# TuragaLab/flybody

Measured on AMD Instinct MI355X. Metric: env steps/sec (whole node), walk_imitation 4096-batch random-action rollout, higher is better.
Workload: dtype f64

## Files before the change

flybody_amd/csrc/fb_constraint.hpp:

```cpp
#pragma once
#include "fb_types.hpp"
#include "fb_math.hpp"
#include "fb_smooth.hpp"
#include "fb_newton.hpp"

#define JIDX(side, s, r) (((r)*2 + (side))*FB_MAXCH + (s))
#define MINIMP ((real)0.0001)
#define MAXIMP ((real)0.9999)

template <typename real>
FBD real get_impedance(const real* si, real pos, real margin) {
  real s0 = fmin(MAXIMP, fmax(MINIMP, si[0])), s1 = fmin(MAXIMP, fmax(MINIMP, si[1]));
  real s2 = fmax((real)0, si[2]), s3 = fmin(MAXIMP, fmax(MINIMP, si[3])), s4 = fmax((real)1, si[4]);
  if (s0 == s1 || s2 <= FB_MINV) return (real)0.5*(s0 + s1);
  real x = fabs((pos - margin)/s2);
  if (x >= 1) return s1;
  if (x <= 0) return s0;
  real y;
  if (s4 == 1) y = x;
  else if (s4 == 2) y = (x <= s3) ? x*x/s3 : 1 - (1 - x)*(1 - x)/(1 - s3);
  else if (x <= s3) y = pow(x, s4) / pow(s3, s4 - 1);
  else y = 1 - pow(1 - x, s4) / pow(1 - s3, s4 - 1);
  return s0 + y*(s1 - s0);
}
// ... 55 lines not shown
  real coff[3] = {0, 0, 0}, cfr[9] = {0, 0, 0, 0, 0, 0, 0, 0, 0};
  if (lane < ncon) {
    p = w.con_pair()[lane];
    dist = w.con_dist()[lane];
#pragma unroll
    for (int k = 0; k < 3; k++) coff[k] = w.con_pos()[3*lane + k] - w.com()[k];
#pragma unroll
    for (int k = 0; k < 9; k++) cfr[k] = w.con_frame()[9*lane + k];
    incl = M.pair_margin[p] - M.pair_gap[p];
    if (dist < incl) dim = (M.pair_condim[p] == 1) ? 1 : 3;
  }
  int adr = nlimit + wave_excl_scan(dim, lane);
  bool over = dim > 0 && adr + dim > FB_MAXEFC_;
  unsigned long long ob = __ballot(over);
  int nefc = nlimit + wave_sum_i(dim);
  if (ob) {
    int first = __ffsll((long long)ob) - 1;
    nefc = __shfl(adr, first, 64);
    if (lane >= first) dim = 0;
  }
  if (lane < ncon) { w.con_efc()[lane] = dim ? adr : -1; w.con_dim()[lane] = dim; }
  int b1 = 0, b2 = 0;
  if (dim) {
    { const int pb = M.pair_body[p]; b1 = pb & 0xffff; b2 = pb >> 16; }
    real K, B, imp;
    kbi(M, M.pair_solref + 2*p, M.pair_solimp + 5*p, dist, incl, false, K, B, imp);
    real tran = M.body_invweight0[2*b1] + M.body_invweight0[2*b2];
    real R0 = fmax(FB_MINV, (1 - imp)*tran/imp);
    const real* fr = M.pair_friction + 5*p;
    real R1 = R0 / fmax(FB_MINV, M.impratio);
    real mu = fr[0]*sqrt(R1/R0);
    real R2 = R1*fr[0]*fr[0]/(fr[1]*fr[1]);
    const int l1 = M.body_chlen[b1], l2 = M.body_chlen[b2];
    const int eA = l1 > 0 ? M.body_chain[b1*FB_MAXCH + l1 - 1] : -1, eB = l2 > 0 ? M.body_chain[b2*FB_MAXCH + l2 - 1] : -1;
    for (int k = 0; k < dim; k++) {
      int r = adr + k;
      w.efc_type()[r] = (dim == 1) ? CN_FRICTIONLESS : CN_ELLIPTIC; w.efc_id()[r] = lane;
      w.efc_bA()[r] = b1; w.efc_bB()[r] = b2;
      w.efc_lA()[r] = l1; w.efc_lB()[r] = l2;
      w.efc_pos()[r] = dist; w.efc_margin()[r] = incl;
      w.efc_K()[r] = (k == 0) ? K : (real)0; w.efc_B()[r] = B; w.efc_imp()[r] = imp;
      const real Rk = (k == 0) ? R0 : (k == 1 ? R1 : R2);
      w.efc_R()[r] = Rk; w.efc_D()[r] = (real)1 / Rk;
      w.efc_mu()[r] = mu;
      w.efc_k()[r] = k; w.efc_s1()[r] = (dim == 1) ? (real)1 : fr[0]; w.efc_s2()[r] = (dim == 1) ? (real)1 : fr[1];
      w.efc_eA()[r] = eA; w.efc_eB()[r] = eB;
    }
  }
  {
    const int cb1 = b1, cb2 = b2;
    const int nitem = ncon*(2*FB_MAXCH);
    for (int t0 = 0; t0 < nitem; t0 += FB_WAVE) {
      const int t = t0 + lane;
      const int c = min(t/(2*FB_MAXCH), FB_WAVE - 1), rem = t - c*(2*FB_MAXCH), side = rem >= FB_MAXCH ? 1 : 0, sl = rem - side*FB_MAXCH;
      const int cdim = __shfl(dim, c, 64), cadr = __shfl(adr, c, 64);
      const int sb1 = __shfl(cb1, c, 64), sb2 = __shfl(cb2, c, 64);
      const int body = side ? sb2 : sb1;
      real off[3], fr[9];
#pragma unroll
      for (int k = 0; k < 3; k++) off[k] = __shfl(coff[k], c, 64);
#pragma unroll
      for (int k = 0; k < 9; k++) fr[k] = __shfl(cfr[k], c, 64);
      if (t < nitem && cdim && sl < M.body_chlen[body]) {
        const int len = M.body_chlen[body];
        const int dof = M.body_chain[body*FB_MAXCH + sl];
        real jp[3] = {0, 0, 0};
        const FB_LDS real* cp = w.lLD + 6*((sl < len) ? dof : 0);
        real cd[6];
#pragma unroll
        for (int k = 0; k < 6; k++) cd[k] = cp[k];
        if (sl < len) {
          real tt[3]; cross3(tt, cd, off);
          jp[0] = cd[3] + tt[0]; jp[1] = cd[4] + tt[1]; jp[2] = cd[5] + tt[2];
        }
        const real sgn = side ? (real)1 : (real)-1;
        for (int k = 0; k < cdim; k++) w.efc_J()[JIDX(side, sl, cadr + k)] = sgn*dot3(fr + 3*k, jp);
      }
    }
  }
  if (lane == 0) {
    if (nefc > w.istate()[IS_MAX_NEFC]) w.istate()[IS_MAX_NEFC] = nefc;
    if (nefc > 32) w.istate()[IS_N_GT32]++;
    if (nefc > 64) w.istate()[IS_N_GT64]++;
    w.istate()[IS_NEFC] = nefc; w.istate()[IS_NLIMIT] = nlimit; if (ob || nlimit > FB_MAXEFC_) { atomicOr(w.istate() + IS_WARN, (int)WARN_EFC_CAP); atomicOr(w.istate() + IS_WARN_EVER, (int)WARN_EFC_CAP); } }
  SYNC();
}

#define ARIDX(r, c) ((r)*((r) + 1)/2 + (c))

template <typename real, typename ARP>
FB_STAGE_B void d_build_AR(const DevModel<real>& M, const WS<real>& w, ARP AR, int nefc, int lane);

template <typename real>
FBD void project_row(const DevModel<real>& M, const WS<real>& w, int side, int r, int body, int len, const FB_LDS real* sd, real* y) {
  int chain[FB_MAXCH], rowadr[FB_MAXCH];
  load_chain(M, body, chain);
#pragma unroll
  for (int s = 0; s < FB_MAXCH; s++) { y[s] = (s < len) ? w.efc_J()[JIDX(side, s, r)] : (real)0; rowadr[s] = (int)w.lmadr()[chain[s]] + s; }
  const int chmax = M.chmax;
#pragma unroll
  for (int s = FB_MAXCH - 1; s >= 1; s--) {
    if (s < chmax) {
      const FB_LDS real* row = w.lLD + rowadr[s];
#pragma unroll
      for (int t = 0; t < s; t++) y[t] -= row[-t] * y[s];
    }
  }
#pragma unroll
  for (int s = 0; s < FB_MAXCH; s++) y[s] = (s < len) ? y[s]*sd[chain[s]] : (real)0;
}

template <int TRUNK, typename real, typename ARP>
FBD void ar_from_registers_t(const DevModel<real>& M, const WS<real>& w, ARP AR, int nefc, int lane, const real* yA, const real* yB, int bA, int bB, int lA, int lB) {
  const bool valid = lane < nefc;
  const int c = lane;
  const int* common = M.body_common; const int nb = M.nbody;
  int rbA = rdlane(bA, 0), rbB = rdlane(bB, 0);
  int cAA = common[rbA*nb + bA], cAB = common[rbA*nb + bB], cBA = common[rbB*nb + bA], cBB = common[rbB*nb + bB];
  const real Rc = valid ? w.efc_R()[c] : (real)0;
  real tr[TRUNK > 0 ? TRUNK : 1];
#pragma unroll
  for (int s = 0; s < TRUNK; s++) tr[s] = yA[s] + yB[s];
  for (int r = 0; r < nefc; r++) {
    int rlA = rdlane(lA, r), rlB = rdlane(lB, r);
    int cmAA = min(min(cAA, lA), rlA), cmAB = min(min(cAB, lB), rlA), cmBA = min(min(cBA, lA), rlB), cmBB = min(min(cBB, lB), rlB);
    if (r + 1 < nefc) {
      rbA = rdlane(bA, r + 1); rbB = rdlane(bB, r + 1);
      cAA = common[rbA*nb + bA]; cAB = common[rbA*nb + bB]; cBA = common[rbB*nb + bA]; cBB = common[rbB*nb + bB];
    }
    real acc = 0;
#pragma unroll
    for (int s = 0; s < TRUNK; s++) acc += rdlane(tr[s], r)*tr[s];
#pragma unroll
    for (int s0 = 0; s0 < FB_MAXCH; s0 += 4) {
      if (s0 + 4 > TRUNK && s0 < rlA) {
#pragma unroll
        for (int s = s0; s < s0 + 4; s++) if (s >= TRUNK) { real yr = rdlane(yA[s], r); if (s < cmAA) acc += yr*yA[s]; if (s < cmAB) acc += yr*yB[s]; }
      }
    }
#pragma unroll
    for (int s0 = 0; s0 < FB_MAXCH; s0 += 4) {
      if (s0 + 4 > TRUNK && s0 < rlB) {
#pragma unroll
        for (int s = s0; s < s0 + 4; s++) if (s >= TRUNK) { real yr = rdlane(yB[s], r); if (s < cmBA) acc += yr*yA[s]; if (s < cmBB) acc += yr*yB[s]; }
      }
    }
    if (valid && c <= r) {
      if (c == r) acc += Rc;
      AR[ARIDX(r, c)] = acc;
    }
  }
  SYNC();
}
template <typename real, typename ARP>
FBD void ar_from_registers(const DevModel<real>& M, const WS<real>& w, ARP AR, int nefc, int lane, const real* yA, const real* yB, int bA, int bB, int lA, int lB) {
  if (uniform_int(M.ntrunk) == FB_MAXTRUNK) ar_from_registers_t<FB_MAXTRUNK>(M, w, AR, nefc, lane, yA, yB, bA, bB, lA, lB);
  else
  ar_from_registers_t<0>(M, w, AR, nefc, lane, yA, yB, bA, bB, lA, lB);
}

template <typename real>
__device__ __forceinline__ void d_project_constraint(const DevModel<real>& M, const WS<real>& w, int lane) {
  int nefc = w.istate()[IS_NEFC];
  if (nefc == 0) return;
  FB_LDS real* sd = w.lx();
  for (int i = lane; i < M.nv; i += FB_WAVE) sd[i] = sqrt(w.lLD[w.lmadr()[i]]);
  SYNC();
  if (nefc <= FB_WAVE) {
    real yA[FB_MAXCH], yB[FB_MAXCH];
    int bA = 0, bB = 0, lA = 0, lB = 0;
    if (lane < nefc) { bA = w.efc_bA()[lane]; bB = w.efc_bB()[lane]; lA = w.efc_lA()[lane]; lB = w.efc_lB()[lane]; }
    project_row(M, w, 0, lane < nefc ? lane : 0, bA, lA, sd, yA);
    project_row(M, w, 1, lane < nefc ? lane : 0, bB, lB, sd, yB);
    if (nefc <= LdsCfg<real>::AR_ROWS) ar_from_registers(M, w, w.lAR(), nefc, lane, yA, yB, bA, bB, lA, lB);
    else ar_from_registers(M, w, w.AR(), nefc, lane, yA, yB, bA, bB, lA, lB);
    return;
  }
  for (int base = 0; base < nefc; base += FB_WAVE) {
    int r = base + lane;
    if (r < nefc) {
      for (int side = 0; side < 2; side++) {
        int body = side ? w.efc_bB()[r] : w.efc_bA()[r];
        int len = side ? w.efc_lB()[r] : w.efc_lA()[r];
        real y[FB_MAXCH];
        project_row(M, w, side, r, body, len, sd, y);
#pragma unroll
        for (int s = 0; s < FB_MAXCH; s++) w.efc_Y()[JIDX(side, s, r)] = y[s];
      }
    }
  }
  SYNC();
  const WS<real> wc = w;
  d_build_AR(M, wc, w.AR(), nefc, lane);
}

template <typename real, typename ARP>
FB_STAGE_B void d_build_AR(const DevModel<real>& M_, const WS<real>& w_, ARP AR, int nefc, int lane) {
  const DevModel<real>& M = as_constant(M_); const WS<real> w = ws_uniform(w_, M);
  for (int cbase = 0; cbase < nefc; cbase += FB_WAVE) {
    int c = cbase + lane;
    bool valid = c < nefc;
    real yA[FB_MAXCH], yB[FB_MAXCH];
    int bA = 0, bB = 0, lA = 0, lB = 0;
    if (valid) { bA = w.efc_bA()[c]; bB = w.efc_bB()[c]; lA = w.efc_lA()[c]; lB = w.efc_lB()[c]; }
#pragma unroll
    for (int s = 0; s < FB_MAXCH; s++) {
      yA[s] = valid ? w.efc_Y()[JIDX(0, s, c)] : (real)0;
      yB[s] = valid ? w.efc_Y()[JIDX(1, s, c)] : (real)0;
    }
    if (nefc <= FB_WAVE) {
      const int* common = M.body_common; const int nb = M.nbody;
      int rbA = rdlane(bA, 0), rbB = rdlane(bB, 0);
      int cAA = common[rbA*nb + bA], cAB = common[rbA*nb + bB], cBA = common[rbB*nb + bA], cBB = common[rbB*nb + bB];
      for (int r = 0; r < nefc; r++) {
        int rlA = rdlane(lA, r), rlB = rdlane(lB, r);
        int cmAA = min(min(cAA, lA), rlA), cmAB = min(min(cAB, lB), rlA), cmBA = min(min(cBA, lA), rlB), cmBB = min(min(cBB, lB), rlB);
        if (r + 1 < nefc) {
          rbA = rdlane(bA, r + 1); rbB = rdlane(bB, r + 1);
          cAA = common[rbA*nb + bA]; cAB = common[rbA*nb + bB]; cBA = common[rbB*nb + bA]; cBB = common[rbB*nb + bB];
        }
        real acc = 0;
#pragma unroll
        for (int s = 0; s < FB_MAXCH; s++) {
          if (s < rlA) { real yr = rdlane(yA[s], r); if (s < cmAA) acc += yr*yA[s]; if (s < cmAB) acc += yr*yB[s]; }
        }
#pragma unroll
        for (int s = 0; s < FB_MAXCH; s++) {
          if (s < rlB) { real yr = rdlane(yB[s], r); if (s < cmBA) acc += yr*yA[s]; if (s < cmBB) acc += yr*yB[s]; }
        }
        if (valid && c <= r) {
          if (c == r) acc += w.efc_R()[r];
          AR[ARIDX(r, c)] = acc;
        }
      }
    } else
    for (int r = 0; r < nefc; r++) {
      real acc = 0;
      for (int side = 0; side < 2; side++) {
        int rb = side ? w.efc_bB()[r] : w.efc_bA()[r];
        int rl = side ? w.efc_lB()[r] : w.efc_lA()[r];
        if (rl == 0) continue;
        int cmA = min(min(M.body_common[rb*M.nbody + bA], lA), rl);
        int cmB = min(min(M.body_common[rb*M.nbody + bB], lB), rl);
#pragma unroll
        for (int s = 0; s < FB_MAXCH; s++) {
          if (s < rl) {
            real yr = w.efc_Y()[JIDX(side, s, r)];
            if (s < cmA) acc += yr*yA[s];
            if (s < cmB) acc += yr*yB[s];
          }
        }
      }
      if (valid && c <= r) {
        if (c == r) acc += w.efc_R()[r];
        AR[ARIDX(r, c)] = acc;
      }
    }
  }
  SYNC();
}

template <typename real>
__device__ __forceinline__ void d_actuation(const DevModel<real>& M, const WS<real>& w, int lane) {
  FB_LDS real* qf = w.lx();
  FB_LDS real* Lc = w.lLD;
  for (int i = lane; i < M.nv; i += FB_WAVE) qf[i] = 0;
  SYNC_LDS();
  const int ncon_l = w.istate()[IS_NCON];
  int cb1 = 0, cb2 = 0, cp = 0;
  real coff[3] = {0, 0, 0}, cnrm[3] = {0, 0, 0};
  constexpr int NCD = (6*FB_MAXNV + FB_WAVE - 1)/FB_WAVE;
  real cdr[NCD];
  if (M.nadh > 0) {
    cp = w.con_pair()[lane];
#pragma unroll
    for (int k = 0; k < 3; k++) { coff[k] = w.con_pos()[3*lane + k]; cnrm[k] = w.con_frame()[9*lane + k]; }
#pragma unroll
    for (int j = 0; j < NCD; j++) { const int i = lane + FB_WAVE*j; cdr[j] = i < 6*M.nv ? w.cdof()[i] : (real)0; }
  }
  for (int i = lane; i < M.nu; i += FB_WAVE) {
    const int limited = M.act_ctrllimited[i], aa = M.act_actadr[i], tt = M.act_trntype[i], wn = M.act_wn[i], la = M.act_lenadr[i];
    const int biastype = M.act_biastype[i], flimited = M.act_forcelimited[i];
    const real c_lo = M.act_ctrlrange[2*i], c_hi = M.act_ctrlrange[2*i+1], dyn = M.act_dynprm[i], gain = M.act_gainprm[3*i];
    const real b0 = M.act_biasprm[3*i], b1 = M.act_biasprm[3*i+1], b2 = M.act_biasprm[3*i+2], f_lo = M.act_forcerange[2*i], f_hi = M.act_forcerange[2*i+1];
    int wd[FB_MAXWRAP]; real wc[FB_MAXWRAP], qv[FB_MAXWRAP];
#pragma unroll
    for (int k = 0; k < FB_MAXWRAP; k++) { wd[k] = M.act_wdof[FB_MAXWRAP*i + k]; wc[k] = M.act_wcoef[FB_MAXWRAP*i + k]; }
    real ctrl = w.ctrl()[i];
    const real actv = w.act()[aa >= 0 ? aa : 0];
#pragma unroll
    for (int k = 0; k < FB_MAXWRAP; k++) qv[k] = w.qvel()[wd[k]];
    const real lq = w.qpos()[tt == TRN_JOINT ? la : 0];
    const real lt = w.ten_length()[tt == TRN_TENDON ? la : 0];
    if (limited) ctrl = clampr(ctrl, c_lo, c_hi);
    real input = ctrl;
    if (aa >= 0) {
      w.act_dot()[aa] = (ctrl - actv) / fmax(FB_MINV, dyn);
      input = actv;
    }
    real length = 0, vel = 0;
    if (tt == TRN_JOINT) length = lq;
    else if (tt == TRN_TENDON) length = lt;
#pragma unroll
    for (int k = 0; k < FB_MAXWRAP; k++) if (k < wn) vel += wc[k]*qv[k];
    real force = gain*input;
    if (biastype == 1) force += b0 + b1*length + b2*vel;
    if (flimited) force = clampr(force, f_lo, f_hi);
    w.act_force()[i] = force;
#pragma unroll
    for (int k = 0; k < FB_MAXWRAP; k++) if (k < wn) qf[wd[k]] = wc[k]*force;
  }
// ... 637 lines not shown
```

flybody_amd/csrc/fb_engine.hip:

```cpp
#ifdef FB_EMULATE
#include "emu/hip_emu.hpp"
#else
#include <hip/hip_runtime.h>
#endif
#include <algorithm>
#include <cmath>
#include <cstdio>
#include <cstdlib>
#include <cstring>
#include <map>
#include <stdexcept>
#include <string>
#include <vector>
#if defined(FB_EMULATE) && defined(FB_STATS)
extern "C" { long long fb_stats[64]; }
#endif

#include "../../include/flybody_engine.h"
#include "fb_step.hpp"
#include "fb_ik.hpp"
#include "fb_inverse.hpp"

static thread_local std::string g_err;
static int fail(const std::string& s) { g_err = s; return -1; }
// ... 660 lines not shown
    int key = iarena[(size_t)(j*nq + xcc)*nint + off_nefc]; key = key < 0 ? 0 : (key > 255 ? 255 : key);
    atomicAdd(&s_hist[255 - key], 1);
  }
  __syncthreads();
  if (tid == 0) { int acc = 0; for (int k = 0; k < 256; k++) { int h = s_hist[k]; s_hist[k] = acc; acc += h; } }
  __syncthreads();
  for (int j = tid; j < cnt; j += FB_ORDER_THREADS) {
    const int e = j*nq + xcc;
    int key = iarena[(size_t)e*nint + off_nefc]; key = key < 0 ? 0 : (key > 255 ? 255 : key);
    order[xcc*stride + atomicAdd(&s_hist[255 - key], 1)] = e;
  }
}

FB_HD __forceinline__ void fb_philox4x32_10(uint32_t c0, uint32_t c1, uint32_t c2, uint32_t c3, uint32_t k0, uint32_t k1, uint32_t* out) {
  for (int r = 0; r < 10; r++) {
    const uint64_t p0 = (uint64_t)0xD2511F53u*c0, p1 = (uint64_t)0xCD9E8D57u*c2;
    const uint32_t n0 = (uint32_t)(p1 >> 32) ^ c1 ^ k0, n1 = (uint32_t)p1, n2 = (uint32_t)(p0 >> 32) ^ c3 ^ k1, n3 = (uint32_t)p0;
    c0 = n0; c1 = n1; c2 = n2; c3 = n3;
    k0 += 0x9E3779B9u; k1 += 0xBB67AE85u;
  }
  out[0] = c0; out[1] = c1; out[2] = c2; out[3] = c3;
}
__global__ void __launch_bounds__(FB_WAVE) k_actions(float* out, const int* env_ids, int n_env, int nact, uint32_t seed_lo, uint32_t seed_hi, int step, int env_id_base, int dist) {
  const int ngrp = (nact + 3)/4;
  const int t = blockIdx.x*FB_WAVE + threadIdx.x;
  if (t >= n_env*ngrp) return;
  const int e = t / ngrp, g = t - e*ngrp;
  const int gid = env_ids ? env_ids[e] : env_id_base + e;
  uint32_t r[4];
  fb_philox4x32_10((uint32_t)step, (uint32_t)gid, (uint32_t)g, (uint32_t)dist, seed_lo, seed_hi, r);
  float v[4];
  if (dist == 1) {
    for (int k = 0; k < 4; k++) v[k] = ((float)(r[k] >> 8) + 0.5f)*(2.0f/16777216.0f) - 1.0f;
  } else {
    for (int k = 0; k < 4; k += 2) {
      const float u1 = ((float)(r[k] >> 8) + 0.5f)*(1.0f/16777216.0f), u2 = ((float)(r[k + 1] >> 8) + 0.5f)*(1.0f/16777216.0f);
      const float rad = sqrtf(-2.0f*logf(u1)), ang = 6.28318530717958647692f*u2;
      v[k] = rad*cosf(ang); v[k + 1] = rad*sinf(ang);
    }
    for (int k = 0; k < 4; k++) v[k] = fminf(1.0f, fmaxf(-1.0f, v[k]));
  }
  for (int k = 0; k < 4; k++) if (4*g + k < nact) out[(size_t)e*nact + 4*g + k] = v[k];
}

extern "C" int fb_random_actions(float* action, const int32_t* env_ids, int n_env, int nact, uint64_t seed, int step, int env_id_base, int dist, void* stream) {
  if (!action || n_env <= 0 || nact <= 0 || (dist != 0 && dist != 1)) return fail("fb_random_actions: bad arguments");
  const int total = n_env*((nact + 3)/4);
  hipLaunchKernelGGL(k_actions, dim3((total + FB_WAVE - 1)/FB_WAVE), dim3(FB_WAVE), 0, (hipStream_t)stream, action, (const int*)env_ids, n_env, nact,
                     (uint32_t)(seed & 0xffffffffu), (uint32_t)(seed >> 32), step, env_id_base, dist);
  HIPCHK(hipGetLastError());
  return 0;
}

struct fb_batch {
  const fb_model* m;
  int n_env, device, precision, nobs;
  WSOff off;
  void* rarena = nullptr; int* iarena = nullptr;
  float *obs = nullptr, *reward = nullptr, *discount = nullptr; int* step_type = nullptr;
  int* d_ids = nullptr;
  int* sched = nullptr;
  int *cost = nullptr, *order = nullptr; bool order_valid = false, reorder = true, use_prio = true, ticket_order = true;
  int *tick = nullptr, *done = nullptr, *sched_err = nullptr, *torder = nullptr; int nq = 0, slots = 0; bool tickets = false;
  unsigned xcc_mask = 0; std::vector<void*> probed_streams; unsigned* probe_word = nullptr;
  void* park = nullptr;
  std::vector<void*> allocs;
  DevModel<double> M64; DevModel<float> M32;
  void* dM = nullptr;
  std::vector<char> dM_copy;
  void *ref_qpos = nullptr, *ref_qvel = nullptr;
  bool have_ref = false, have_wbpg = false;
  hipEvent_t ev0 = nullptr, ev1 = nullptr; int timed_launches = 0; bool timing = false;
  std::vector<hipEvent_t> lev;
  double* ik_err = nullptr; int* ik_steps = nullptr;
  void* ik_buf = nullptr; size_t ik_buf_bytes = 0;
  double* inv_qfrc = nullptr; double* inv_cforce = nullptr;
  void *qfrc_applied = nullptr, *xfrc_applied = nullptr;
};

template <typename real, typename T, typename P>
static int upload(fb_batch* b, const T* src, size_t n, P* dst) {
  std::vector<real> tmp(n ? n : 1);
  for (size_t k = 0; k < n; k++) tmp[k] = (real)src[k];
  void* p;
  HIPCHK(hipMalloc(&p, tmp.size()*sizeof(real)));
  HIPCHK(hipMemcpy(p, tmp.data(), tmp.size()*sizeof(real), hipMemcpyHostToDevice));
  b->allocs.push_back(p);
  *dst = (const real*)p;
  return 0;
}
template <typename P>
static int upload_i(fb_batch* b, const int* src, size_t n, P* dst) {
  void* p;
  HIPCHK(hipMalloc(&p, (n ? n : 1)*sizeof(int)));
  if (n) HIPCHK(hipMemcpy(p, src, n*sizeof(int), hipMemcpyHostToDevice));
  else HIPCHK(hipMemset(p, 0, sizeof(int)));
  b->allocs.push_back(p);
  *dst = (const int*)p;
  return 0;
}

template <typename F>
static auto with_model(fb_batch* b, F&& f) { return b->precision == 64 ? f(b->M64) : f(b->M32); }
static size_t real_size(fb_batch* b) { return with_model(b, [](auto& M) { return sizeof(M.timestep); }); }

static int sync_model(fb_batch* b) {
  return with_model(b, [&](auto& M) {
    if (!b->dM) HIPCHK(hipMalloc(&b->dM, sizeof(M)));
    const char* h = (const char*)&M;
    if (b->dM_copy.empty() || memcmp(h, b->dM_copy.data(), sizeof(M)) != 0) {
      HIPCHK(hipDeviceSynchronize());
      HIPCHK(hipMemcpy(b->dM, h, sizeof(M), hipMemcpyHostToDevice));
      b->dM_copy.assign(h, h + sizeof(M));
    }
    return 0;
  });
}

template <typename T>
static int alloc_zeroed_once(T** p, size_t bytes) {
  if (!*p) { HIPCHK(hipMalloc((void**)p, bytes)); HIPCHK(hipMemset(*p, 0, bytes)); }
  return 0;
}

static int alloc_obs(fb_batch* b, int nobs) {
  (void)hipFree(b->obs); b->obs = nullptr;
  HIPCHK(hipMalloc((void**)&b->obs, (size_t)b->n_env*nobs*sizeof(float)));
  HIPCHK(hipMemset(b->obs, 0, (size_t)b->n_env*nobs*sizeof(float)));
  b->nobs = nobs;
  return 0;
}

template <typename real>
static int build_devmodel(fb_batch* b, DevModel<real>& M) {
  const fb_model* m = b->m;
  memset(&M, 0, sizeof(M));
  M.nq = m->nq; M.nv = m->nv; M.nbody = m->nbody; M.njnt = m->njnt; M.ngeom = m->ngeom; M.nsite = m->nsite;
  M.nu = m->nu; M.na = m->na; M.ntendon = m->ntendon; M.npair = m->npair; M.nM = m->nM; M.nsubstep = m->nsubstep;
  M.nobsjnt = m->nobsjnt; M.napp = m->napp; M.nforce = m->nforce; M.ntouch = m->ntouch;
  M.site_thorax = m->i("sensor_site_thorax")[0]; M.nadh = (int)m->adh_act.size();
  M.iterations = m->i("opt_iterations")[0]; M.noslip_iterations = m->i("opt_noslip_iterations")[0];
  M.solver = (m->has("opt_solver", 1) && m->i("opt_solver")[0] == FB_SOLVER_PGS) ? FB_SOLVER_PGS : FB_SOLVER_NEWTON;
  M.timestep = (real)m->d("opt_timestep")[0]; M.control_timestep = (real)m->d("opt_control_timestep")[0];
  for (int k = 0; k < 3; k++) M.grav[k] = (real)m->d("opt_gravity")[k];
  M.density = (real)m->d("opt_density")[0]; M.viscosity = (real)m->d("opt_viscosity")[0];
  M.impratio = (real)m->d("opt_impratio")[0]; M.tolerance = (real)m->d("opt_tolerance")[0];
  {
    std::vector<double> rb; const double* r_ = m->d("geom_rbound");
    for (int g = 0; g < m->ngeom; g++) if (r_[g] > 0) rb.push_back(r_[g]);
    std::sort(rb.begin(), rb.end());
    M.vl_delta = (rb.empty() || m->npair <= 4*FB_WAVE) ? (real)0 : (real)(FB_VL_SCALE*rb[rb.size()/2]);
    { const char* e_ = getenv("FB_NO_NEIGHBOUR_LIST"); if (e_ && e_[0] == '1') M.vl_delta = 0; }
  }
  M.noslip_tolerance = (real)m->d("opt_noslip_tolerance")[0]; M.meaninertia = (real)m->d("stat_meaninertia")[0];
  M.totalmass = (real)m->totalmass;
  size_t c;
#define UI(field, name) { const int* s_ = m->i(name, &c); if (upload_i(b, s_, c, &M.field)) return -1; }
#define UV(field, vec) { if (upload_i(b, m->vec.data(), m->vec.size(), &M.field)) return -1; }
#define UD(field, name) { const double* s_ = m->d(name, &c); if (upload<real>(b, s_, c, &M.field)) return -1; }
  UI(body_parent, "body_parent") UI(body_dofadr, "body_dofadr")
  UV(body_nsub, body_nsub) UV(body_depth, body_depth) UV(body_chlen, body_chlen) UV(body_chain, body_chain) UV(body_common, body_common)
  UI(jnt_type, "jnt_type") UI(jnt_qposadr, "jnt_qposadr") UI(jnt_dofadr, "jnt_dofadr") UI(jnt_bodyid, "jnt_bodyid") UI(jnt_limited, "jnt_limited")
  UI(dof_bodyid, "dof_bodyid") UI(dof_jntid, "dof_jntid") UI(dof_Madr, "dof_Madr") UV(dof_depth, dof_depth)
  UV(dof_ndesc, dof_ndesc) UV(body_fluid_geom, body_fluid_geom) UV(sens_body, sens_body) M.nsensbody = (int)m->sens_body.size();
  UV(dof_jump, dof_jump) UV(dof_vbef, dof_vbef) UV(body_veldof, body_veldof)
  UV(dof_cl, dof_cl) UV(dof_gen, dof_gen) UV(gen_k, gen_k) UV(gen_m, gen_m) UV(fwd_tab, fwd_tab) UV(fwd_pack, fwd_pack) UV(fac_w, fac_w) UV(fac_band, fac_band) UV(fac_dof, fac_dof) M.ntrunk = m->ntrunk; M.prefix_split = m->prefix_split;
  { int dmax = 0, d2 = 1 << 20; for (int bq = 1; bq < m->nbody; bq++) { dmax = std::max(dmax, m->body_depth[bq]); if (bq >= FB_WAVE) d2 = std::min(d2, m->body_depth[bq]); } M.fk_dmax = dmax; M.fk2_dlo = d2; }
  { int cm = 0; for (int bq = 0; bq < m->nbody; bq++) cm = std::max(cm, m->body_chlen[bq]); M.chmax = cm; }
  {
    std::vector<int> second(FB_WAVE, -1);
    bool ok = m->nbody > FB_WAVE && m->nbody <= 2*FB_WAVE && getenv("FB_NO_FK_MERGE") == nullptr;
    for (int bq = FB_WAVE; ok && bq < m->nbody; bq++) {
      int pick = -1;
      for (int l = 0; l < FB_WAVE && pick < 0; l++) if (second[l] < 0 && (l == 0 || m->body_depth[l] < m->body_depth[bq])) pick = l;
      if (pick < 0) ok = false; else second[pick] = bq;
    }
    M.fk_second = nullptr;
    if (ok && upload_i(b, second.data(), second.size(), &M.fk_second)) return -1;
  }
  UI(wing_act_idx, "wing_action_idx")
  if (m->has("leg_joints", 1)) { UI(leg_jnt, "leg_joints") M.nlegjnt = (int)c; for (size_t k = 0; k < c; k++) if (m->i("leg_joints")[k] < 0 || m->i("leg_joints")[k] >= m->njnt) return fail("fb_batch_create: leg_joints out of range"); }
  else { UV(leg_jnt, adh_act) M.nlegjnt = 0; }
  M.task = m->task_id; M.user_idx = m->i("user_action_idx")[0]; M.nact = m->nu + (M.user_idx >= 0 ? 1 : 0);
  for (int k = 0; k < 3; k++) M.com_offset[k] = (real)m->d("com_offset")[k];
  M.nlevel = m->nlevel;
  UI(geom_type, "geom_type") UI(geom_bodyid, "geom_bodyid") UI(site_bodyid, "site_bodyid") UI(site_type, "site_type")
  UI(tendon_adr, "tendon_adr") UI(tendon_num, "tendon_num")
  UI(act_trntype, "actuator_trntype") UI(act_trnid, "actuator_trnid") UI(act_dyntype, "actuator_dyntype") UI(act_biastype, "actuator_biastype")
  UI(act_ctrllimited, "actuator_ctrllimited") UI(act_forcelimited, "actuator_forcelimited") UI(act_actadr, "actuator_actadr")
  UV(adh_act, adh_act) UI(action_to_ctrl, "action_to_ctrl")
  UV(wrap_qadr, wrap_qadr) UV(act_wn, act_wn) UV(act_wdof, act_wdof) UV(act_lenadr, act_lenadr)
  if (upload<real>(b, m->act_wcoef.data(), m->act_wcoef.size(), &M.act_wcoef)) return -1;
  UI(pair_geom1, "pair_geom1") UI(pair_geom2, "pair_geom2") UI(pair_condim, "pair_condim")
  UV(pair_word, pair_word) UV(pair_body, pair_body) UV(plane_geoms, plane_geoms)
  { const int* gt_ = m->i("geom_type"); int np_ = 0; for (int g = 0; g < m->ngeom; g++) np_ += gt_[g] == GEOM_PLANE; M.nplane = np_; }
  UI(obs_jnt, "observable_joints") UI(app_sites, "appendage_sites") UI(force_sites, "sensor_force_sites") UI(touch_sites, "sensor_touch_sites") UI(wing_jnt, "wing_jnt")
  UD(body_mass, "body_mass")
  UD(body_inertia, "body_inertia") UD(body_invweight0, "body_invweight0")
  if (upload<real>(b, m->body_box.data(), m->body_box.size(), &M.body_box)) return -1;
  if (upload<real>(b, m->geom_box.data(), m->geom_box.size(), &M.geom_box)) return -1;
  if (upload<real>(b, m->body_rec.data(), m->body_rec.size(), &M.body_rec)) return -1;
  UD(jnt_axis, "jnt_axis") UD(jnt_stiffness, "jnt_stiffness") UD(jnt_range, "jnt_range") UD(jnt_solref, "jnt_solref")
  UD(jnt_solimp, "jnt_solimp") UD(jnt_margin, "jnt_margin") UD(qpos0, "qpos0") UD(qpos_spring, "qpos_spring")
  UD(dof_armature, "dof_armature") UD(dof_damping, "dof_damping") UD(dof_invweight0, "dof_invweight0")
  UD(geom_pos, "geom_pos") UD(geom_quat, "geom_quat") UD(geom_size, "geom_size") UD(geom_rbound, "geom_rbound") UD(geom_fluid, "geom_fluid")
  UD(site_pos, "site_pos") UD(site_quat, "site_quat") UD(site_size, "site_size") UD(wrap_coef, "wrap_coef")
  UD(act_dynprm, "actuator_dynprm") UD(act_gainprm, "actuator_gainprm") UD(act_biasprm, "actuator_biasprm") UD(act_ctrlrange, "actuator_ctrlrange") UD(act_forcerange, "actuator_forcerange")
  UD(pair_friction, "pair_friction") UD(pair_solref, "pair_solref") UD(pair_solimp, "pair_solimp") UD(pair_margin, "pair_margin") UD(pair_gap, "pair_gap")
#undef UI
#undef UV
#undef UD
  return 0;
}

template <typename real>
static void compute_offsets(const DevModel<real>& M, WSOff& o) {
  uint32_t r = 0, i = 0;
  auto al = [](uint32_t v) { return (v + 15u) & ~15u; };
#define X(name, n) o.name = r; r = al(r + (uint32_t)(n));
  FB_WS_REAL(X)
#undef X
#define X(name, n) o.name = i; i = al(i + (uint32_t)(n));
  FB_WS_INT(X)
#undef X
  o.nreal = (r + 15u) & ~15u; o.nint = (i + 15u) & ~15u;
}

static int batch_create_impl(fb_batch* b);

extern "C" int fb_batch_create(const fb_model* m, int n_env, int device, int precision, fb_batch** out) {
  if (!out) return fail("fb_batch_create: null output pointer");
  *out = nullptr;
  if (!m || n_env <= 0) return fail("fb_batch_create: bad arguments");
  if (precision != 32 && precision != 64) return fail("fb_batch_create: precision must be 32 or 64");
  int ndev = 0;
  if (hipGetDeviceCount(&ndev) != hipSuccess || ndev <= 0) return fail("fb_batch_create: no HIP device available (the engine has no CPU fallback)");
  if (device < 0 || device >= ndev) return fail("fb_batch_create: bad device index");
  HIPCHK(hipSetDevice(device));
  fb_batch* b = new fb_batch();
  b->m = m; b->n_env = n_env; b->device = device; b->precision = precision;
  int rc;
  try { rc = batch_create_impl(b); } catch (const std::exception& e_) { rc = fail(std::string("fb_batch_create: ") + e_.what()); }
  if (rc != 0) { std::string keep = g_err; fb_batch_destroy(b); g_err = keep; return rc; }
  *out = b;
  return 0;
}

static int batch_create_impl(fb_batch* b) {
  const fb_model* m = b->m; const int n_env = b->n_env;
  if (with_model(b, [&](auto& M) { if (build_devmodel(b, M)) return -1; compute_offsets(M, b->off); M.off = b->off; return 0; })) return -1;
  const size_t rs = real_size(b);
  HIPCHK(hipMalloc(&b->rarena, (size_t)n_env*b->off.nreal*rs));
  HIPCHK(hipMemset(b->rarena, 0, (size_t)n_env*b->off.nreal*rs));
  HIPCHK(hipMalloc((void**)&b->iarena, (size_t)n_env*b->off.nint*sizeof(int)));
  HIPCHK(hipMemset(b->iarena, 0, (size_t)n_env*b->off.nint*sizeof(int)));
  HIPCHK(hipMalloc((void**)&b->reward, n_env*sizeof(float)));
  HIPCHK(hipMalloc((void**)&b->discount, n_env*sizeof(float)));
  HIPCHK(hipMalloc((void**)&b->step_type, n_env*sizeof(int)));
  HIPCHK(hipMalloc((void**)&b->d_ids, n_env*sizeof(int)));
  HIPCHK(hipMalloc((void**)&b->sched, FB_NSCHED*sizeof(int)));
  HIPCHK(hipMalloc((void**)&b->cost, n_env*sizeof(int)));
  HIPCHK(hipMemset(b->cost, 0, n_env*sizeof(int)));
  HIPCHK(hipMalloc((void**)&b->order, n_env*sizeof(int)));
  { const char* e_ = getenv("FB_NO_REORDER"); b->reorder = !(e_ && e_[0] == '1'); b->ticket_order = b->reorder; }
  {
#ifdef FB_EMULATE
    b->nq = 1; b->slots = 2;
#else
    hipDeviceProp_t prop; HIPCHK(hipGetDeviceProperties(&prop, b->device));
    if (with_model(b, [&](auto& M) {
          using real = decltype(M.timestep);
          int nb = 0;
          HIPCHK(hipOccupancyMaxActiveBlocksPerMultiprocessor(&nb, k_fly<real>, FB_WAVE*LdsCfg<real>::EPB, 0));
          int nbf = 0;
          HIPCHK(hipOccupancyMaxActiveBlocksPerMultiprocessor(&nbf, k_step_forces<real>, FB_WAVE*LdsCfg<real>::EPB, 0));
          b->slots = std::min(nb, nbf)*prop.multiProcessorCount*LdsCfg<real>::EPB;
          return 0; })) return -1;
    unsigned* dmask; unsigned hmask = 0;
    HIPCHK(hipMalloc((void**)&dmask, sizeof(unsigned))); HIPCHK(hipMemset(dmask, 0, sizeof(unsigned)));
    hipLaunchKernelGGL(k_probe_xcc, dim3(4096), dim3(FB_WAVE), 0, 0, dmask);
    HIPCHK(hipMemcpy(&hmask, dmask, sizeof(unsigned), hipMemcpyDeviceToHost)); HIPCHK(hipFree(dmask));
    int nqq = __builtin_popcount(hmask);
    b->nq = (nqq > 0 && hmask == (1u << nqq) - 1u) ? nqq : 0;
    b->xcc_mask = hmask;
    if (strncmp(prop.gcnArchName, "gfx942", 6) != 0 && strncmp(prop.gcnArchName, "gfx950", 6) != 0) b->nq = 0;
    if (const char* e_ = getenv("FB_TICKET_SLOTS")) b->slots = atoi(e_);
#endif
    HIPCHK(hipMalloc((void**)&b->tick, 16*16*sizeof(int)));
    HIPCHK(hipMalloc((void**)&b->done, n_env*sizeof(int)));
    HIPCHK(hipMalloc((void**)&b->torder, (size_t)(n_env + 16)*sizeof(int)));
    HIPCHK(hipMalloc((void**)&b->sched_err, sizeof(int)));
    HIPCHK(hipMemset(b->sched_err, 0, sizeof(int)));
    HIPCHK(hipMalloc((void**)&b->probe_word, sizeof(unsigned)));
    b->tickets = b->nq > 0 && b->slots > 0 && n_env > b->slots && getenv("FB_NO_TICKETS") == nullptr;
  }
  b->use_prio = getenv("FB_NO_PRIO") == nullptr;
  HIPCHK(hipMemset(b->reward, 0, n_env*sizeof(float)));
  HIPCHK(hipMemset(b->discount, 0, n_env*sizeof(float)));
  HIPCHK(hipMemset(b->step_type, 0, n_env*sizeof(int)));
  if (with_model(b, [&](auto& M) {
        std::vector<decltype(M.timestep)> rows((size_t)n_env*m->nq);
        const double* q0 = m->d("qpos0");
        for (int e = 0; e < n_env; e++) std::copy_n(q0, m->nq, rows.data() + (size_t)e*m->nq);
        HIPCHK(hipMemcpy2D((char*)b->rarena + (size_t)b->off.qpos*rs, (size_t)b->off.nreal*rs, rows.data(), (size_t)m->nq*rs, (size_t)m->nq*rs, n_env, hipMemcpyHostToDevice));
        return 0; })) return -1;
  b->nobs = 0;
// ... 601 lines not shown
```

flybody_amd/csrc/fb_types.hpp:

```cpp
#pragma once
#ifdef FB_EMULATE
#include "emu/hip_emu.hpp"
#else
#include <hip/hip_runtime.h>
#endif
#include <stdint.h>

#if defined(FB_EMULATE) && defined(FB_STATS)
extern "C" { extern long long fb_stats[64]; }
#define FB_STAT(k) (fb_stats[k]++)
#else
#define FB_STAT(k) do {} while (0)
#endif

#define FB_WAVE 64
#define FB_EPB 4
#define FB_MAXCH 20
#define FB_MAXGEN 16
#define FB_LDS_SCRATCH 1216
#define FB_LGEN 6
#define FB_BODYREC 40
#define FB_MAXTRUNK 6
#define FB_FSLOT 18
#define FB_FGEN 2
#define FB_MAXDEPTH 10
#define FB_MAXCON_ 64
#define FB_MAXEFC_ 192
#define FB_NSENS 33
#define FB_NWS_VECS 18
#define FB_NPROF 56
#define FB_NSCHED 64
#define FB_MAXWRAP 8
#define FB_MAXNM 1280
#define FB_MAXNV 112
#define FB_NJUMP 5

enum { JNT_FREE = 0, JNT_BALL = 1, JNT_HINGE = 3 };
enum { GEOM_PLANE = 0, GEOM_SPHERE = 2, GEOM_CAPSULE = 3, GEOM_ELLIPSOID = 4, GEOM_CYLINDER = 5 };
enum { TRN_JOINT = 0, TRN_TENDON = 3, TRN_BODY = 5 };
enum { DYN_NONE = 0, DYN_FILTER = 2, DYN_FILTEREXACT = 3 };
enum { CN_LIMIT = 0, CN_FRICTIONLESS = 1, CN_ELLIPTIC = 2 };
enum { IS_STEP = 0, IS_RESET_NEXT = 1, IS_STEP_TYPE = 2, IS_NCON = 3, IS_NEFC = 4, IS_NITER = 5, IS_NLIMIT = 6, IS_NCAND = 7,
       IS_WB_STEP = 8, IS_WB_FREQ = 9, IS_EPISODE = 10, IS_DS_OFF = 11, IS_DS_LEN = 12, IS_EPSTEPS = 13, IS_PRIO = 14, IS_WARN = 15, IS_WARN_EVER = 16,
       IS_MAX_NCON = 17, IS_MAX_NEFC = 18, IS_N_GT32 = 19, IS_N_GT64 = 20,
       IS_VL_OK = 21, IS_VL_N = 22, IS_VL_SKIP = 23,
       IS_N = 24 };
#define FB_VL_SCALE 0.5
#define FB_VLMAX 448
enum { WARN_CONTACT_CAP = 1, WARN_EFC_CAP = 2, WARN_SOLVER_MAXITER = 4, WARN_CCD_MAXITER = 8, WARN_SCHED_WAIT = 16, WARN_SOLVER_FALLBACK = 32 };


#if defined(__HIP_DEVICE_COMPILE__) && !defined(FB_EMULATE)
#define FB_GLOBAL __attribute__((address_space(1)))
#define FB_CONST __attribute__((address_space(4)))
#else
#define FB_GLOBAL
#define FB_CONST
#endif
#ifdef FB_EMULATE
#define FB_HD
#else
#define FB_HD __host__ __device__
#endif
template <typename T> struct GP {
  FB_GLOBAL T* p;
  FB_HD __forceinline__ operator T*() const { return (T*)p; }
  FB_HD __forceinline__ GP& operator=(T* q) { p = (FB_GLOBAL T*)q; return *this; }
};

#define FB_WS_REAL(X) \
  X(qpos, M.nq) X(qvel, M.nv) X(act, M.na + 1) X(ctrl, M.nu) X(qacc, M.nv) X(qacc_ws, M.nv) X(act_dot, M.na + 1) \
  X(sens, FB_NSENS) X(sens_acc, FB_NSENS) X(simtime, 1) X(wbfreq, 1) X(dsshift, 2) X(rfac, 6) \
  X(xpos, 3*M.nbody) X(xquat, 4*M.nbody)  \
  X(xaxis, 3*M.njnt)  X(gxpos, 3*M.ngeom) X(gxmat, 9*M.ngeom) X(sxpos, 3*M.nsite) X(sxmat, 9*M.nsite) X(com, 4) \
  X(cinert, 10*M.nbody) X(cdof, 6*M.nv) X(cvel, 6*M.nbody) \
  X(qM, M.nM) X(qLD, M.nM) \
  X(qfrc_bias, M.nv) X(qfrc_passive, M.nv) X(qfrc_actuator, M.nv) X(qfrc_smooth, M.nv) X(qacc_smooth, M.nv) \
  X(qfrc_constraint, M.nv) X(ten_length, M.ntendon + 1) X(act_force, M.nu) \
  X(con_dist, FB_MAXCON_) X(con_pos, 3*FB_MAXCON_) X(con_frame, 9*FB_MAXCON_) \
  X(efc_J, 2*FB_MAXCH*FB_MAXEFC_) \
  X(efc_pos, FB_MAXEFC_) X(efc_margin, FB_MAXEFC_) X(efc_R, FB_MAXEFC_) X(efc_D, FB_MAXEFC_) X(efc_K, FB_MAXEFC_) \
  X(efc_B, FB_MAXEFC_) X(efc_imp, FB_MAXEFC_) X(efc_aref, FB_MAXEFC_) X(efc_b, FB_MAXEFC_) X(efc_force, FB_MAXEFC_) \
  X(efc_vel, FB_MAXEFC_) X(efc_mu, FB_MAXEFC_) X(efc_jar, FB_MAXEFC_) X(efc_s1, FB_MAXEFC_) X(efc_s2, FB_MAXEFC_)  \
  X(cacc, 6*M.nbody) X(cfrc, 6*M.nbody) X(cfrc_ext, 6*M.nbody) X(cabias, 6*M.nbody) \
   \
  X(efc_Y, 2*FB_MAXCH*FB_MAXEFC_) X(AR, FB_MAXEFC_*(FB_MAXEFC_ + 1))  \
  X(nws, FB_NWS_VECS*FB_MAXEFC_)  \
  X(vl_pos, 3*M.ngeom)

#define FB_WS_INT(X) \
  X(istate, IS_N) X(prof, 2*FB_NPROF) X(con_pair, FB_MAXCON_) X(con_efc, FB_MAXCON_) X(con_dim, FB_MAXCON_) X(cand, 2*FB_MAXCON_ + 64) \
  X(efc_type, FB_MAXEFC_) X(efc_id, FB_MAXEFC_) X(efc_bA, FB_MAXEFC_) X(efc_bB, FB_MAXEFC_) X(efc_lA, FB_MAXEFC_) X(efc_lB, FB_MAXEFC_) \
  X(efc_k, FB_MAXEFC_)  X(efc_eA, FB_MAXEFC_) X(efc_eB, FB_MAXEFC_)  \
  X(vl_list, FB_VLMAX)

struct WSOff {
#define X(name, n) uint32_t name;
  FB_WS_REAL(X)
  FB_WS_INT(X)
#undef X
  uint32_t nreal, nint;
};

template <typename real>
struct DevModel {
  int nq, nv, nbody, njnt, ngeom, nsite, nu, na, ntendon, npair, nM, nsubstep;
  int nobsjnt, napp, nforce, ntouch, site_thorax, nadh;
  int iterations, noslip_iterations, solver;
  real timestep, control_timestep, grav[3], density, viscosity, impratio, tolerance, noslip_tolerance, meaninertia, totalmass;
  real vl_delta;
  GP<const int> body_parent, body_dofadr, body_nsub, body_depth;
  GP<const int> body_chlen;
  GP<const int> body_chain;
  GP<const int> body_common;
  GP<const int> jnt_type, jnt_qposadr, jnt_dofadr, jnt_bodyid, jnt_limited;
  GP<const int> dof_bodyid, dof_jntid, dof_Madr, dof_depth;
  GP<const int> dof_ndesc;
  int nlevel;
  GP<const int> dof_cl;
  GP<const int> dof_gen;
  GP<const int> gen_k, gen_m;
  GP<const int> fwd_tab;
  GP<const int> fwd_pack;
  GP<const int> fac_w;
  GP<const int> fac_band;
  GP<const int> fac_dof;
  int ntrunk;
  int prefix_split;
  int chmax;
  int fk_dmax, fk2_dlo;
  const int* fk_second;
  GP<const int> geom_type, geom_bodyid, site_bodyid, site_type;
  GP<const int> tendon_adr, tendon_num;
  GP<const int> act_trntype, act_trnid, act_dyntype, act_biastype, act_ctrllimited, act_forcelimited, act_actadr;
  GP<const int> adh_act;
  GP<const int> wrap_qadr;
  GP<const int> act_wn, act_wdof, act_lenadr;
  GP<const real> act_wcoef;
  GP<const int> action_to_ctrl;
  GP<const int> pair_geom1, pair_geom2, pair_condim;
  GP<const int> pair_body;
  GP<const int> pair_word;
  GP<const int> plane_geoms; int nplane;
  GP<const int> obs_jnt, app_sites, force_sites, touch_sites, wing_jnt;
  GP<const int> dof_jump;
  GP<const int> dof_vbef;
  GP<const int> body_veldof;
  GP<const int> sens_body; int nsensbody;
  GP<const real> body_mass, body_inertia, body_invweight0, body_box;
  GP<const real> body_rec;
  GP<const real> jnt_axis, jnt_stiffness, jnt_range, jnt_solref, jnt_solimp, jnt_margin;
  GP<const real> qpos0, qpos_spring, dof_armature, dof_damping, dof_invweight0;
  GP<const real> geom_pos, geom_quat, geom_size, geom_rbound, geom_fluid;
  GP<const real> geom_box;
  GP<const real> site_pos, site_quat, site_size;
  GP<const real> wrap_coef;
  GP<const real> act_dynprm, act_gainprm, act_biasprm, act_ctrlrange, act_forcerange;
  GP<const real> pair_friction, pair_solref, pair_solimp, pair_margin, pair_gap;
  GP<const real> ref_qpos, ref_qvel;
  int T, future_steps, episode_steps, nobs;
  real terminal_com_dist, time_limit;
  int task, nact, user_idx; unsigned seed;
  GP<const int> wing_act_idx, body_fluid_geom;
  real com_offset[3];
  GP<const real> wb_traj, wb_phase, wb_freqs; GP<const int> wb_offset; int wb_nfreq;
  real wb_base_freq, wb_rel_range, wb_rate;
  GP<const real> ds_qpos, ds_qvel, ds_r2s, ds_jq;
  GP<const int> ds_offset, ds_jid, ds_sid, ds_select;
  int ds_nj, ds_ns, ds_ntraj, ds_nselect, ds_env_base, max_episode_steps;
  int ds_random_start;
  GP<const int> leg_jnt; int nlegjnt;
  WSOff off;
};

#ifdef FB_EMULATE
#define FB_LDS
#else
#define FB_LDS __attribute__((address_space(3)))
#endif

#ifndef FB_F64_DENSE
#define FB_F64_DENSE 0
#endif
template <typename real> struct LdsCfg {
  static constexpr bool F64 = sizeof(real) == 8;
  static constexpr int EPB = F64 ? (FB_F64_DENSE ? 4 : 1) : FB_EPB;
  static constexpr int AR_ROWS = F64 ? (FB_F64_DENSE ? 23 : 43) : 46;
  static constexpr int AR_ELEMS = AR_ROWS*(AR_ROWS + 1)/2;
  static constexpr int POOL = FB_LDS_SCRATCH + AR_ELEMS + FB_MAXNV;
  static constexpr int WAVES_PER_SIMD = F64 ? (FB_F64_DENSE ? 3 : 2) : 4;
  static constexpr int wide_rows() { int r = AR_ROWS; while ((r + 1)*(r + 2)/2 <= FB_LDS_SCRATCH + AR_ELEMS && r + 1 <= FB_WAVE) r++; return r; }
  static constexpr int WIDE_ROWS = wide_rows();
};

struct LdsTab {
  uint8_t depth[FB_MAXNV], cl[FB_MAXNV], gen[FB_MAXNV + 2*FB_WAVE];
  uint16_t madr[FB_MAXNV + 1];
  uint32_t gk[FB_LGEN*FB_MAXCH], gm[FB_LGEN*FB_MAXCH*2];
};

template <typename real>
struct WS {
  FB_LDS real* lLD;
  const FB_LDS LdsTab* lt;
  __device__ __forceinline__ FB_LDS real* lAR() const { return lLD + FB_LDS_SCRATCH; }
  __device__ __forceinline__ FB_LDS real* lx() const { return lLD + FB_LDS_SCRATCH + LdsCfg<real>::AR_ELEMS; }
  __device__ __forceinline__ const FB_LDS uint8_t* ldepth() const { return lt->depth; }
  __device__ __forceinline__ const FB_LDS uint8_t* lcl() const { return lt->cl; }
  __device__ __forceinline__ const FB_LDS uint8_t* lgen() const { return lt->gen; }
  __device__ __forceinline__ const FB_LDS uint16_t* lmadr() const { return lt->madr; }
  __device__ __forceinline__ const FB_LDS uint32_t* lgk() const { return lt->gk; }
  __device__ __forceinline__ const FB_LDS uint32_t* lgm() const { return lt->gm; }
  FB_GLOBAL real* rb; FB_GLOBAL int* ib; const FB_CONST WSOff* o;
#define X(name, n) __device__ __forceinline__ real* name() const { return (real*)(rb + o->name); }
  FB_WS_REAL(X)
#undef X
#define X(name, n) __device__ __forceinline__ int* name() const { return (int*)(ib + o->name); }
  FB_WS_INT(X)
#undef X
};
```

Before: 843,900.

## Compute constraint AR matrix with one lane per lower-triangle entry

Adds an alternative A·R assembly path where each wavefront lane computes one packed lower-triangular entry (row/col decoded via sqrt), gathering row and column Jacobian chain values through cross-lane shuffles, instead of the previous per-row/column loop. Trunk contributions are pre-summed per lane and chain blocks are skipped wave-uniformly via ballot masks. It is enabled by default with an env var to disable. This aims to use all lanes for the triangle rather than leaving lanes idle for c>r, at the cost of more cross-lane reads and index arithmetic.

```diff
diff --git a/flybody_amd/csrc/fb_constraint.hpp b/flybody_amd/csrc/fb_constraint.hpp
--- a/flybody_amd/csrc/fb_constraint.hpp
+++ b/flybody_amd/csrc/fb_constraint.hpp
@@ -231,11 +231,78 @@
   }
   SYNC();
 }
+template <int TRUNK, typename real, typename ARP>
+FBD void ar_entry_lanes_t(const DevModel<real>& M, const WS<real>& w, ARP AR, int nefc, int lane, const real* yA, const real* yB, int bA, int bB, int lA, int lB) {
+  const int* common = M.body_common; const int nb = M.nbody;
+  const real Rl = w.efc_R()[lane];
+  const int bodies = bA | (bB << 16), lens = lA | (lB << 8);
+  real tr[TRUNK > 0 ? TRUNK : 1];
+#pragma unroll
+  for (int s = 0; s < TRUNK; s++) tr[s] = yA[s] + yB[s];
+  unsigned any = 0;
+#pragma unroll
+  for (int g = 0; g < FB_MAXCH/4; g++) any |= (__ballot(lA > 4*g) != 0 ? 1u << g : 0u) | (__ballot(lB > 4*g) != 0 ? 0x100u << g : 0u);
+  any = (unsigned)uniform_int((int)any);
+  const int nent = nefc*(nefc + 1)/2;
+  for (int p0 = 0; p0 < nent; p0 += FB_WAVE) {
+    const int p = p0 + lane;
+    const bool valid = p < nent;
+    const int pp = valid ? p : 0;
+    int r = (int)((sqrtf((float)(8*pp + 1)) - 1.0f)*0.5f);
+    r -= (r*(r + 1)/2 > pp) ? 1 : 0;
+    r += ((r + 1)*(r + 2)/2 <= pp) ? 1 : 0;
+    const int c = pp - r*(r + 1)/2;
+    const int rbod = nw_lane_i(bodies, r), cbod = nw_lane_i(bodies, c), rlen = nw_lane_i(lens, r), clen = nw_lane_i(lens, c);
+    const int rbA = rbod & 0xffff, rbB = rbod >> 16, cbA = cbod & 0xffff, cbB = cbod >> 16;
+    const int rlA = rlen & 0xff, rlB = rlen >> 8, clA = clen & 0xff, clB = clen >> 8;
+    const int cmAA = min(min(common[rbA*nb + cbA], clA), rlA), cmAB = min(min(common[rbA*nb + cbB], clB), rlA);
+    const int cmBA = min(min(common[rbB*nb + cbA], clA), rlB), cmBB = min(min(common[rbB*nb + cbB], clB), rlB);
+    const real Rr = nw_lane(Rl, r);
+    real acc = 0;
+    {
+      real tr_r[TRUNK > 0 ? TRUNK : 1], tr_c[TRUNK > 0 ? TRUNK : 1];
+#pragma unroll
+      for (int s = 0; s < TRUNK; s++) { tr_r[s] = nw_lane(tr[s], r); tr_c[s] = nw_lane(tr[s], c); }
+#pragma unroll
+      for (int s = 0; s < TRUNK; s++) acc += tr_r[s]*tr_c[s];
+    }
+#pragma unroll
+    for (int s0 = 0; s0 < FB_MAXCH; s0 += 4) {
+      if (s0 + 4 > TRUNK && ((any >> (s0/4)) & 1u)) {
+        real yr[4], ya[4], yb[4];
+#pragma unroll
+        for (int s = s0; s < s0 + 4; s++) if (s >= TRUNK) { yr[s - s0] = nw_lane(yA[s], r); ya[s - s0] = nw_lane(yA[s], c); yb[s - s0] = nw_lane(yB[s], c); }
+#pragma unroll
+        for (int s = s0; s < s0 + 4; s++) if (s >= TRUNK) { if (s < cmAA) acc += yr[s - s0]*ya[s - s0]; if (s < cmAB) acc += yr[s - s0]*yb[s - s0]; }
+      }
+    }
+#pragma unroll
+    for (int s0 = 0; s0 < FB_MAXCH; s0 += 4) {
+      if (s0 + 4 > TRUNK && ((any >> (8 + s0/4)) & 1u)) {
+        real yr[4], ya[4], yb[4];
+#pragma unroll
+        for (int s = s0; s < s0 + 4; s++) if (s >= TRUNK) { yr[s - s0] = nw_lane(yB[s], r); ya[s - s0] = nw_lane(yA[s], c); yb[s - s0] = nw_lane(yB[s], c); }
+#pragma unroll
+        for (int s = s0; s < s0 + 4; s++) if (s >= TRUNK) { if (s < cmBA) acc += yr[s - s0]*ya[s - s0]; if (s < cmBB) acc += yr[s - s0]*yb[s - s0]; }
+      }
+    }
+    if (valid) {
+      if (c == r) acc += Rr;
+      AR[p] = acc;
+    }
+  }
+  SYNC();
+}
 template <typename real, typename ARP>
 FBD void ar_from_registers(const DevModel<real>& M, const WS<real>& w, ARP AR, int nefc, int lane, const real* yA, const real* yB, int bA, int bB, int lA, int lB) {
-  if (uniform_int(M.ntrunk) == FB_MAXTRUNK) ar_from_registers_t<FB_MAXTRUNK>(M, w, AR, nefc, lane, yA, yB, bA, bB, lA, lB);
-  else
-  ar_from_registers_t<0>(M, w, AR, nefc, lane, yA, yB, bA, bB, lA, lB);
+  const bool entry = uniform_int(M.ar_entry_lanes) != 0;
+  if (uniform_int(M.ntrunk) == FB_MAXTRUNK) {
+    if (entry) ar_entry_lanes_t<FB_MAXTRUNK>(M, w, AR, nefc, lane, yA, yB, bA, bB, lA, lB);
+    else ar_from_registers_t<FB_MAXTRUNK>(M, w, AR, nefc, lane, yA, yB, bA, bB, lA, lB);
+  } else {
+    if (entry) ar_entry_lanes_t<0>(M, w, AR, nefc, lane, yA, yB, bA, bB, lA, lB);
+    else ar_from_registers_t<0>(M, w, AR, nefc, lane, yA, yB, bA, bB, lA, lB);
+  }
 }
 
 template <typename real>
diff --git a/flybody_amd/csrc/fb_engine.hip b/flybody_amd/csrc/fb_engine.hip
--- a/flybody_amd/csrc/fb_engine.hip
+++ b/flybody_amd/csrc/fb_engine.hip
@@ -836,6 +836,8 @@
     M.vl_delta = (rb.empty() || m->npair <= 4*FB_WAVE) ? (real)0 : (real)(FB_VL_SCALE*rb[rb.size()/2]);
     { const char* e_ = getenv("FB_NO_NEIGHBOUR_LIST"); if (e_ && e_[0] == '1') M.vl_delta = 0; }
   }
+  M.ar_entry_lanes = 1;
+  { const char* e_ = getenv("FB_NO_AR_ENTRY_LANES"); if (e_ && e_[0] == '1') M.ar_entry_lanes = 0; }
   M.noslip_tolerance = (real)m->d("opt_noslip_tolerance")[0]; M.meaninertia = (real)m->d("stat_meaninertia")[0];
   M.totalmass = (real)m->totalmass;
   size_t c;
diff --git a/flybody_amd/csrc/fb_types.hpp b/flybody_amd/csrc/fb_types.hpp
--- a/flybody_amd/csrc/fb_types.hpp
+++ b/flybody_amd/csrc/fb_types.hpp
@@ -109,6 +109,7 @@
   int iterations, noslip_iterations, solver;
   real timestep, control_timestep, grav[3], density, viscosity, impratio, tolerance, noslip_tolerance, meaninertia, totalmass;
   real vl_delta;
+  int ar_entry_lanes;
   GP<const int> body_parent, body_dofadr, body_nsub, body_depth;
   GP<const int> body_chlen;
   GP<const int> body_chain;
```

Result: faster. 855,300, median of 6 (+1.4%).
